# nextpyp/spr_pick

Hardware: AMD Instinct MI355X
Metric: train_patches_per_sec (higher is better)
Workload: dtype f32; 1 GPU; BASELINE configs[1]: ssdn --noise_style gaussian --noise_value var, joint mode, 64x64 patches from 4 synthetic 1024x1024 micrographs, batch 32 per GPU, alpha 0.75, tau 0.01, Adam; fp32 MFMA convolutions (Winograd F(2x2,3x3) for the wide 3x3 layers); per_gpu_batch=32, global_batch=32, patch=64, parallelism=single GPU

## Files before the change

### spr_pick_amd/csrc/gemm1x1.hip

```cpp
#include "gemm1x1.h"

#include <type_traits>

#include "conv_dev.h"

namespace {

constexpr int kTP = 256;
constexpr int kXS = kTP + 16;
constexpr int kKC = 32;
constexpr int kLdw = sprk::kGemm1x1Ldw;
constexpr int kWInstr = kKC * kLdw / 256;
static_assert(kKC * kLdw % 256 == 0 && kXS % 32 == 16 && kLdw % 32 == 16, "LDS layout");

struct G1Args {
    const float *x, *wT, *scp, *shp;
    float *y;
    int N, K, Cn, HW;
    int rows, nblkN;
    int act, hasSc, hasSh;
    int steps, nch, c0last;
    int tilesPerImg, nTiles, nh, xcd;
};

template <int NB>
__global__ __launch_bounds__(256) void gemm1x1_kernel(const G1Args a) {
    extern __shared__ __attribute__((aligned(16))) float smem[];
    constexpr int NTT = NB * 6;
    constexpr int stageFloats = kKC * kXS + NB * kKC * kLdw;
    const int tid = threadIdx.x, lane = tid & 63;
    const int wave = __builtin_amdgcn_readfirstlane(tid >> 6);
    const int l15 = lane & 15, lq = lane >> 4;
    const int G = gridDim.x;

    auto decode = [&](int r, int &t, int &h) {
        const int b = blockIdx.x;
        if (a.xcd) {
            const int j = b >> 3;
            h = j % a.nh;
            t = r * (G / a.nh) + (j / a.nh) * 8 + (b & 7);
        } else {
            const int it = r * G + b;
            t = it / a.nh;
            h = it - t * a.nh;
        }
        t = __builtin_amdgcn_readfirstlane(t);
        h = __builtin_amdgcn_readfirstlane(h);
        return t < a.nTiles;
    };
    const rsrc_t wr = make_rsrc(a.wT);
    auto issue = [&](int t, int h, int ci, int b) {
        const int n = __builtin_amdgcn_readfirstlane(t / a.tilesPerImg), p0 = (t - n * a.tilesPerImg) * kTP;
        float *xs = smem + b * stageFloats;
        float *ws = xs + kKC * kXS;
        const rsrc_t xr = make_rsrc(a.x + (long)n * a.K * a.HW);
        const int xv = min(p0 + lane * 4, a.HW - 4) * 4;
        const int r0 = ci * kKC;
#pragma unroll
        for (int i = 0; i < kKC / 4; ++i) {
            const int r = r0 + wave + 4 * i;
            const int ch = r < a.K ? r : a.c0last;
            bdma16(xr, xv, ch * a.HW * 4, xs + (wave + 4 * i) * kXS);
        }
        const int valid = min(kKC, a.rows - r0) * kLdw * 4 - 16;
#pragma unroll
        for (int i0 = 0; i0 < NB * kWInstr; i0 += 4) {
            const int i = min(i0 + wave, NB * kWInstr - 1);
            const int nbi = i / kWInstr, ii = i - nbi * kWInstr;
            const int nb = min(h * NB + nbi, a.nblkN - 1);
            bdma16(wr, min(ii * 1024 + lane * 16, valid), (nb * a.rows + r0) * (kLdw * 4), ws + nbi * (kKC * kLdw) + ii * 256);
        }
    };
    constexpr int kDmaPerWave = kKC / 4 + (NB * kWInstr + 3) / 4;

    int t, h;
    bool ok = decode(0, t, h);
    if (!ok) return;
    issue(t, h, 0, 0);
    const int abase = lds_addr(smem) + (lq * kXS + wave * 64 + l15) * 4;
    const int bbase = lds_addr(smem + kKC * kXS) + (lq * kLdw + l15) * 4;
    int g = 0;
    for (int r = 0; ok; ++r) {
        int tn, hn;
        const bool okn = decode(r + 1, tn, hn);
        const int n = __builtin_amdgcn_readfirstlane(t / a.tilesPerImg), p0 = (t - n * a.tilesPerImg) * kTP;
        const int pix = p0 + wave * 64 + lq * 4;
        float vsc[NTT], vsh[NTT];
#pragma unroll
        for (int j = 0; j < NTT; ++j) {
            const int idx = min(h * (NB * 96) + j * 16 + l15, a.Cn - 1);
            vsc[j] = a.scp[a.hasSc ? idx : 0];
            vsh[j] = a.shp[a.hasSh ? idx : 0];
        }
        f32x4 acc[4][NTT];
#pragma unroll
        for (int mt = 0; mt < 4; ++mt)
#pragma unroll
            for (int j = 0; j < NTT; ++j) acc[mt][j] = f32x4{0.f, 0.f, 0.f, 0.f};

        for (int ci = 0; ci < a.nch; ++ci, ++g) {
            if (ci > 0 || r == 0) asm volatile("s_waitcnt vmcnt(0)" ::: "memory");
            lds_only_barrier();
            const bool lastc = ci + 1 == a.nch;
            const int nq = min(kKC / 4, a.steps - ci * (kKC / 4));
            const int sa = abase + (g & 1) * (stageFloats * 4), sb = bbase + (g & 1) * (stageFloats * 4);
            float a0[4], b0[NTT], a1[4], b1[NTT];
            auto ld = [&](float (&av)[4], float (&bv)[NTT], int q) {
                lds_cfp ap = lds_f(sa + q * (4 * kXS * 4));
#pragma unroll
                for (int mt = 0; mt < 4; ++mt) av[mt] = ap[16 * mt];
                lds_cfp bp = lds_f(sb + q * (4 * kLdw * 4));
#pragma unroll
                for (int j = 0; j < NTT; ++j) bv[j] = bp[(j / 6) * (kKC * kLdw) + 16 * (j % 6)];
            };
            auto mm = [&](const float (&av)[4], const float (&bv)[NTT]) {
#pragma unroll
                for (int mt = 0; mt < 4; ++mt)
#pragma unroll
                    for (int j = 0; j < NTT; ++j)
                        acc[mt][j] = __builtin_amdgcn_mfma_f32_16x16x4f32(av[mt], bv[j], acc[mt][j], 0, 0, 0);
            };
            const int last = nq - 1;
            ld(a0, b0, 0);
            ld(a1, b1, min(1, last));
            {
                const bool own = !lastc || !okn;
                issue(own ? t : tn, own ? h : hn, lastc ? 0 : ci + 1, (g + 1) & 1);
            }
            mm(a0, b0);
#pragma unroll
            for (int i = 0; i < kDmaPerWave; ++i) {
                __builtin_amdgcn_sched_group_barrier(0x008, 4 * NTT / kDmaPerWave, 0);
                __builtin_amdgcn_sched_group_barrier(0x020, 1, 0);
            }
            for (int q = 1; q + 1 < nq; q += 2) {
                ld(a0, b0, q + 1);
                mm(a1, b1);
                ld(a1, b1, min(q + 2, last));
                mm(a0, b0);
            }
            if (!(nq & 1)) mm(a1, b1);
        }
        asm volatile("s_waitcnt vmcnt(0)" ::: "memory");
#pragma unroll
        for (int j = 0; j < NTT; ++j) asm volatile("" : "+v"(vsc[j]), "+v"(vsh[j]));
        auto stores = [&](auto actc) {
            constexpr int ACT = decltype(actc)::value;
#pragma unroll
            for (int j = 0; j < NTT; ++j) {
                const int co = h * (NB * 96) + j * 16 + l15;
                if (co >= a.Cn) continue;
                const float sc = a.hasSc ? vsc[j] : 1.f, sh = vsh[j];
                float *yc = a.y + ((long)n * a.Cn + co) * a.HW + pix;
#pragma unroll
                for (int mt = 0; mt < 4; ++mt) {
                    if (pix + 16 * mt >= a.HW) continue;
                    const f32x4 c = acc[mt][j];
                    float v[4];
#pragma unroll
                    for (int e = 0; e < 4; ++e) v[e] = apply_act(c[e] * sc + sh, ACT);
                    *reinterpret_cast<float4 *>(yc + 16 * mt) = make_float4(v[0], v[1], v[2], v[3]);
                }
            }
        };
        if (a.act == SPRK_ACT_LEAKY)
            stores(std::integral_constant<int, SPRK_ACT_LEAKY>{});
        else if (a.act == SPRK_ACT_RELU)
            stores(std::integral_constant<int, SPRK_ACT_RELU>{});
        else
            stores(std::integral_constant<int, SPRK_ACT_NONE>{});
        t = tn;
        h = hn;
        ok = okn;
    }
}

inline int slabs_per_item(int nblkN) { return nblkN >= 2 ? 2 : 1; }

template <int NB>
int launch(const G1Args &a, int grid, hipStream_t s) {
    const size_t lds = 2 * (size_t)(kKC * kXS + NB * kKC * kLdw) * sizeof(float);
    if (int rc = sprk::lds_optin(gemm1x1_kernel<NB>, lds, "gemm1x1")) return rc;
    hipLaunchKernelGGL(gemm1x1_kernel<NB>, dim3(grid), dim3(256), lds, s, a);
    return SPRK_OK;
}

}

namespace sprk {

std::atomic<long> g_gemm1x1_launches{0};
std::atomic<int> g_gemm1x1_on{1};

bool gemm1x1_fits(int N, int K, int HW) {
    return K >= kGemm1x1MinK && HW >= 4 && HW % 4 == 0 && (long)K * HW * 4 < (1L << 31) &&
           (long)N * cdiv(HW, kTP) < (1L << 28);
}

int gemm1x1_grid(int N, int HW, int nblkN) {
    const int nh = cdiv(nblkN, slabs_per_item(nblkN));
    const long items = (long)N * cdiv(HW, kTP) * nh;
    int G = (int)std::min<long>(items, num_cus());
    if (G >= 8 * nh) G -= G % (8 * nh);
    return std::max(G, 1);
}

int gemm1x1_run(const Gemm1x1Call &c, hipStream_t s) {
    SPRK_REQUIRE(gemm1x1_fits(c.N, c.K, c.HW) && c.ldw == kLdw && c.rows == cdiv(c.K, 16) * 16 && c.nblkN >= 1 &&
                     c.nblkN == cdiv(c.Cn, 96) && (long)c.nblkN * c.rows * kLdw * 4 < (1L << 31),
                 "gemm1x1: call outside the kernel's limits");
    const int NB = slabs_per_item(c.nblkN);
    G1Args a{};
    a.x = c.x; a.wT = c.wT; a.y = c.y;
    a.scp = c.scale ? c.scale : c.zeros;
    a.shp = c.scale ? c.shift : (c.bias ? c.bias : c.zeros);
    a.hasSc = c.scale != nullptr;
    a.hasSh = (c.scale || c.bias) ? 1 : 0;
    a.N = c.N; a.K = c.K; a.Cn = c.Cn; a.HW = c.HW;
    a.rows = c.rows; a.nblkN = c.nblkN;
    a.act = c.act;
    a.steps = cdiv(c.K, 4);
    a.nch = cdiv(a.steps, kKC / 4);
    a.c0last = (c.K - 1) / 16 * 16;
    a.tilesPerImg = cdiv(c.HW, kTP);
    a.nTiles = c.N * a.tilesPerImg;
    a.nh = cdiv(c.nblkN, NB);
    const int grid = gemm1x1_grid(c.N, c.HW, c.nblkN);
    a.xcd = (grid % (8 * a.nh) == 0) ? 1 : 0;
    if (int rc = NB == 2 ? launch<2>(a, grid, s) : launch<1>(a, grid, s)) return rc;
    g_gemm1x1_launches.fetch_add(1, std::memory_order_relaxed);
    return SPRK_OK;
}

}
```

### spr_pick_amd/csrc/mask1x1.hip

```cpp
#include "mask1x1.h"

#include "conv_dev.h"

namespace {

constexpr int kTP = 128;
constexpr int kMaxSteps = 30;
constexpr int kTabEntries = kMaxSteps + 2;

struct M1Args {
    const float *gy, *wT, *mask;
    float *gin;
    int N, K, Cn, HW;
    int CK, R4, rows, ldw;
    int act, steps, tilesPerImg, nTiles;
};

using i32x2 = __attribute__((ext_vector_type(2))) int;
typedef const __attribute__((address_space(3))) i32x2 *lds_ci2p;

template <int NT>
__global__ __launch_bounds__(256) void mask1x1_kernel(const M1Args a) {
    extern __shared__ __attribute__((aligned(16))) float smem[];
    i32x2 *tab = reinterpret_cast<i32x2 *>(smem);
    float *w_lds = smem + kTabEntries * 4 * 2;
    const int wFloats = a.rows * a.ldw;
    float *stage = w_lds + wFloats;
    const int stageFloats = a.K * kTP;

    const int tid = threadIdx.x, lane = tid & 63;
    const int wave = __builtin_amdgcn_readfirstlane(tid >> 6);
    const int l15 = lane & 15, lq = lane >> 4;
    const int nb = blockIdx.y;
    const long HW = a.HW;

    {
        const float *wsrc = a.wT + (long)nb * wFloats;
        const int total4 = wFloats >> 2;
        for (int gi = wave; gi * 64 < total4; gi += 4) {
            const int idx = gi * 64 + lane;
            if (idx < total4) dma16(wsrc + idx * 4, w_lds + gi * 256);
        }
    }
    auto issue = [&](int t, int b) {
        const int n = t / a.tilesPerImg, p0 = (t - n * a.tilesPerImg) * kTP;
        const int chl = lane >> 5;
        const int px = min(p0 + (lane & 31) * 4, a.HW - 4);
        const float *src = a.gy + (long)n * a.K * HW + px;
        float *dst = stage + b * stageFloats;
        for (int c = wave * 2; c < a.K; c += 8) {
            const int ch = c + chl;
            if (ch < a.K) dma16(src + (long)ch * HW, dst + c * kTP);
        }
    };
    int t = blockIdx.x;
    issue(t, 0);
    if (tid < kTabEntries * 4) {
        const int s = min(tid >> 2, a.steps - 1), l = tid & 3;
        int c0 = 0, ci = 0, q = s;
        for (;;) {
            const int nkq = (min(a.CK, a.K - c0) + 3) >> 2;
            if (q < nkq) break;
            q -= nkq;
            c0 += a.CK;
            ++ci;
        }
        const int cke = min(a.CK, a.K - c0), kk = 4 * q + l;
        tab[tid] = i32x2{(c0 + (kk < cke ? kk : 0)) * (kTP * 4), (ci * a.R4 + kk) * (a.ldw * 4)};
    }
    const int abase = lds_addr(stage) + (wave * 32 + l15) * 4;
    const int bbase = lds_addr(w_lds) + l15 * 4;
    lds_ci2p tp = (lds_ci2p)(__SIZE_TYPE__)(unsigned)lds_addr(tab + lq);
    const bool leaky = a.act == SPRK_ACT_LEAKY;

    asm volatile("s_waitcnt vmcnt(0)" ::: "memory");
    for (int i = 0; t < a.nTiles; t += gridDim.x, ++i) {
        lds_only_barrier();
        if (t + (int)gridDim.x < a.nTiles) issue(t + gridDim.x, (i + 1) & 1);
        const int n = t / a.tilesPerImg, p0 = (t - n * a.tilesPerImg) * kTP;
        const int pix = p0 + wave * 32 + lq * 4;
        float4 mk[2][NT];
#pragma unroll
        for (int nt = 0; nt < NT; ++nt) {
            const int co = min(nb * (NT * 16) + nt * 16 + l15, a.Cn - 1);
            const float *mp = a.mask + ((long)n * a.Cn + co) * HW;
#pragma unroll
            for (int mt = 0; mt < 2; ++mt) mk[mt][nt] = *reinterpret_cast<const float4 *>(mp + min(pix + 16 * mt, a.HW - 4));
        }
        f32x4 acc[2][NT];
#pragma unroll
        for (int mt = 0; mt < 2; ++mt)
#pragma unroll
            for (int nt = 0; nt < NT; ++nt) acc[mt][nt] = f32x4{0.f, 0.f, 0.f, 0.f};
        const int sa = abase + (i & 1) * stageFloats * 4;
        float av[2], bv[NT];
        i32x2 e1 = tp[4];
        {
            const i32x2 e0 = tp[0];
            lds_cfp ap = lds_f(sa + e0.x);
            av[0] = ap[0];
            av[1] = ap[16];
            lds_cfp bp = lds_f(bbase + e0.y);
#pragma unroll
            for (int nt = 0; nt < NT; ++nt) bv[nt] = bp[16 * nt];
        }
        for (int s = 0; s < a.steps; ++s) {
            const i32x2 e2 = tp[(s + 2) * 4];
            float an[2], bn[NT];
            lds_cfp ap = lds_f(sa + e1.x);
            an[0] = ap[0];
            an[1] = ap[16];
            lds_cfp bp = lds_f(bbase + e1.y);
#pragma unroll
            for (int nt = 0; nt < NT; ++nt) bn[nt] = bp[16 * nt];
#pragma unroll
            for (int mt = 0; mt < 2; ++mt)
#pragma unroll
                for (int nt = 0; nt < NT; ++nt)
                    acc[mt][nt] = __builtin_amdgcn_mfma_f32_16x16x4f32(av[mt], bv[nt], acc[mt][nt], 0, 0, 0);
            av[0] = an[0];
            av[1] = an[1];
#pragma unroll
            for (int nt = 0; nt < NT; ++nt) bv[nt] = bn[nt];
            e1 = e2;
        }
        asm volatile("s_waitcnt vmcnt(0)" ::: "memory");
#pragma unroll
        for (int nt = 0; nt < NT; ++nt)
#pragma unroll
            for (int mt = 0; mt < 2; ++mt)
                asm volatile("" : "+v"(mk[mt][nt].x), "+v"(mk[mt][nt].y), "+v"(mk[mt][nt].z), "+v"(mk[mt][nt].w));
#pragma unroll
        for (int nt = 0; nt < NT; ++nt) {
            const int co = nb * (NT * 16) + nt * 16 + l15;
            if (co >= a.Cn) continue;
#pragma unroll
            for (int mt = 0; mt < 2; ++mt) {
                if (pix + 16 * mt >= a.HW) continue;
                const f32x4 c = acc[mt][nt];
                const float4 m = mk[mt][nt];
                float4 v = make_float4(c[0] + 0.f, c[1] + 0.f, c[2] + 0.f, c[3] + 0.f);
                v.x = m.x > 0.f ? v.x : (leaky ? v.x * kLeak : 0.f);
                v.y = m.y > 0.f ? v.y : (leaky ? v.y * kLeak : 0.f);
                v.z = m.z > 0.f ? v.z : (leaky ? v.z * kLeak : 0.f);
                v.w = m.w > 0.f ? v.w : (leaky ? v.w * kLeak : 0.f);
                *reinterpret_cast<float4 *>(a.gin + ((long)n * a.Cn + co) * HW + pix + 16 * mt) = v;
            }
        }
    }
}

template <int NT>
int launch(const M1Args &a, dim3 grid, size_t lds, hipStream_t s) {
    if (int rc = sprk::lds_optin(mask1x1_kernel<NT>, lds, "mask1x1")) return rc;
    hipLaunchKernelGGL(mask1x1_kernel<NT>, grid, dim3(256), lds, s, a);
    return SPRK_OK;
}

}

namespace sprk {

int mask1x1_steps(int K, int CK) {
    if (K < 1 || K > kMask1x1MaxK || CK < 1) return 0;
    int steps = 0;
    for (int c0 = 0; c0 < K; c0 += CK) steps += (std::min(CK, K - c0) + 3) >> 2;
    return steps <= kMaxSteps ? steps : 0;
}

int mask1x1_run(const Mask1x1Call &c, hipStream_t s) {
    M1Args a{};
    a.gy = c.gy; a.wT = c.wT; a.mask = c.mask; a.gin = c.gin;
    a.N = c.N; a.K = c.K; a.Cn = c.Cn; a.HW = c.HW;
    a.CK = c.CK; a.R4 = c.R4; a.rows = c.rows; a.ldw = c.ldw;
    a.act = c.act;
    a.steps = mask1x1_steps(c.K, c.CK);
    a.tilesPerImg = cdiv(c.HW, kTP);
    a.nTiles = c.N * a.tilesPerImg;
    SPRK_REQUIRE(a.steps > 0 && c.HW >= 4 && c.HW % 4 == 0 && (long)c.N * a.tilesPerImg < (1L << 30) &&
                     (c.rows * c.ldw) % 4 == 0 && (c.act == SPRK_ACT_LEAKY || c.act == SPRK_ACT_RELU),
                 "mask1x1: call outside the kernel's limits");
    const size_t lds = ((size_t)kTabEntries * 8 + (size_t)c.rows * c.ldw + 2 * (size_t)c.K * kTP) * sizeof(float);
    SPRK_REQUIRE(lds <= 160 * 1024, "mask1x1: %zu bytes of LDS", lds);
    int wgs = std::max(1, num_cus() / c.nblkN);
    if (wgs >= 8) wgs &= ~7;
    const dim3 grid(std::min(a.nTiles, wgs), c.nblkN);
    int rc;
    switch (c.NT) {
        case 1: rc = launch<1>(a, grid, lds, s); break;
        case 2: rc = launch<2>(a, grid, lds, s); break;
        case 3: rc = launch<3>(a, grid, lds, s); break;
        case 4: rc = launch<4>(a, grid, lds, s); break;
        case 6: rc = launch<6>(a, grid, lds, s); break;
        default: set_error("mask1x1: no kernel for %d channel tiles per slab", c.NT); return SPRK_EINVAL;
    }
    if (rc) return rc;
    g_mask1x1_launches.fetch_add(1, std::memory_order_relaxed);
    return SPRK_OK;
}

}
```

Baseline: 2084 patches/s.

## Split 1x1 GEMM and mask kernels across eight waves per workgroup

The gemm1x1 kernel now launches eight waves, with the two halves splitting the output channel tiles, which halves the per-wave accumulator count, and it also seeds the first MFMA with zero instead of clearing accumulators. The mask1x1 kernel halves its pixel tile and runs two independent four-wave groups per workgroup, each with its own double-buffered stage, interleaving tiles and using staggered barriers. The aim is more waves in flight and less register pressure to hide LDS and MFMA latency. The costs are more LDS per block, extra barriers, and B-operand LDS reads repeated across the wave halves. A scratch benchmark script is added.

```diff
diff --git a/scratch/head_waves_bench.py b/scratch/head_waves_bench.py
--- /dev/null
+++ b/scratch/head_waves_bench.py
@@ -0,0 +1,52 @@
+import statistics
+import sys
+
+import torch
+
+from spr_pick_amd import _lib, ops
+
+reps = int(sys.argv[1]) if len(sys.argv) > 1 else 10
+L = _lib.lib()
+S = torch.ops.sprk
+dev = torch.device("cuda:0")
+g = torch.Generator().manual_seed(1)
+N, HW = 64, 64
+
+
+def timed(fn):
+    ts = []
+    for _ in range(reps):
+        a, b = torch.cuda.Event(enable_timing=True), torch.cuda.Event(enable_timing=True)
+        a.record()
+        fn()
+        b.record()
+        torch.cuda.synchronize()
+        ts.append(a.elapsed_time(b) * 1e3)
+    return ts
+
+
+def rnd(*shape, scale=1.0):
+    return (torch.randn(*shape, generator=g) * scale).to(dev)
+
+
+for name, K, Cout, kind in (("gemm1x1 fwd 384->384", 384, 384, "fwd"), ("gemm1x1 fwd 384->96", 384, 96, "fwd"),
+                            ("gemm1x1 bwd 384->384", 384, 384, "bwd"), ("mask1x1 bwd 96->384", 96, 384, "mask")):
+    x = rnd(N, K, HW, HW)
+    if kind == "fwd":
+        w, b = rnd(Cout, K, 1, 1, scale=K ** -0.5), rnd(Cout)
+        geom = ops.make_geom(x, None, w, False, 1, 1, (0, 0, 0, 0))
+        fn = lambda: ops.conv2d_forward(x, None, w, geom, bias=b, act=ops.ACT_LEAKY)
+    else:
+        w = rnd(K, Cout, 1, 1, scale=K ** -0.5)
+        mask = rnd(N, Cout, HW, HW) if kind == "mask" else None
+        geom = ops.make_geom(torch.empty(N, Cout, HW, HW, device=dev), None, w, False, 1, 1, (0, 0, 0, 0))
+        fn = lambda: S.conv2d_bwd_data(x, w, ops.geom_list(geom), mask, ops.ACT_LEAKY if kind == "mask" else ops.ACT_NONE, None)
+    n0 = L.sprk_gemm1x1_launch_count(), L.sprk_mask1x1_launch_count()
+    fn()
+    torch.cuda.synchronize()
+    took = L.sprk_gemm1x1_launch_count() - n0[0], L.sprk_mask1x1_launch_count() - n0[1]
+    ts = timed(fn)
+    print("%-22s launches (gemm1x1, mask1x1) %s  median %.1f us  min %.1f  max %.1f  (%.1f TF at the minimum)" % (
+        name, took, statistics.median(ts), min(ts), max(ts), 2.0 * N * HW * HW * K * Cout / min(ts) * 1e-6), flush=True)
+    del x, w, fn
+    torch.cuda.empty_cache()
diff --git a/spr_pick_amd/csrc/gemm1x1.hip b/spr_pick_amd/csrc/gemm1x1.hip
--- a/spr_pick_amd/csrc/gemm1x1.hip
+++ b/spr_pick_amd/csrc/gemm1x1.hip
@@ -9,9 +9,10 @@
 constexpr int kTP = 256;
 constexpr int kXS = kTP + 16;
 constexpr int kKC = 32;
+constexpr int kNW = 8;
 constexpr int kLdw = sprk::kGemm1x1Ldw;
 constexpr int kWInstr = kKC * kLdw / 256;
-static_assert(kKC * kLdw % 256 == 0 && kXS % 32 == 16 && kLdw % 32 == 16, "LDS layout");
+static_assert(kKC % kNW == 0 && kKC * kLdw % 256 == 0 && kXS % 32 == 16 && kLdw % 32 == 16, "LDS layout");
 
 struct G1Args {
     const float *x, *wT, *scp, *shp;
@@ -24,12 +25,13 @@
 };
 
 template <int NB>
-__global__ __launch_bounds__(256) void gemm1x1_kernel(const G1Args a) {
+__global__ __launch_bounds__(kNW * 64) void gemm1x1_kernel(const G1Args a) {
     extern __shared__ __attribute__((aligned(16))) float smem[];
-    constexpr int NTT = NB * 6;
+    constexpr int NTT = NB * 3;
     constexpr int stageFloats = kKC * kXS + NB * kKC * kLdw;
     const int tid = threadIdx.x, lane = tid & 63;
     const int wave = __builtin_amdgcn_readfirstlane(tid >> 6);
+    const int wq = wave & 3, wh = wave >> 2;
     const int l15 = lane & 15, lq = lane >> 4;
     const int G = gridDim.x;
 
@@ -57,46 +59,42 @@
         const int xv = min(p0 + lane * 4, a.HW - 4) * 4;
         const int r0 = ci * kKC;
 #pragma unroll
-        for (int i = 0; i < kKC / 4; ++i) {
-            const int r = r0 + wave + 4 * i;
+        for (int i = 0; i < kKC / kNW; ++i) {
+            const int r = r0 + wave + kNW * i;
             const int ch = r < a.K ? r : a.c0last;
-            bdma16(xr, xv, ch * a.HW * 4, xs + (wave + 4 * i) * kXS);
+            bdma16(xr, xv, ch * a.HW * 4, xs + (wave + kNW * i) * kXS);
         }
         const int valid = min(kKC, a.rows - r0) * kLdw * 4 - 16;
 #pragma unroll
-        for (int i0 = 0; i0 < NB * kWInstr; i0 += 4) {
+        for (int i0 = 0; i0 < NB * kWInstr; i0 += kNW) {
             const int i = min(i0 + wave, NB * kWInstr - 1);
             const int nbi = i / kWInstr, ii = i - nbi * kWInstr;
             const int nb = min(h * NB + nbi, a.nblkN - 1);
             bdma16(wr, min(ii * 1024 + lane * 16, valid), (nb * a.rows + r0) * (kLdw * 4), ws + nbi * (kKC * kLdw) + ii * 256);
         }
     };
-    constexpr int kDmaPerWave = kKC / 4 + (NB * kWInstr + 3) / 4;
+    constexpr int kDmaPerWave = kKC / kNW + (NB * kWInstr + kNW - 1) / kNW;
 
     int t, h;
     bool ok = decode(0, t, h);
     if (!ok) return;
     issue(t, h, 0, 0);
-    const int abase = lds_addr(smem) + (lq * kXS + wave * 64 + l15) * 4;
-    const int bbase = lds_addr(smem + kKC * kXS) + (lq * kLdw + l15) * 4;
+    const int abase = lds_addr(smem) + (lq * kXS + wq * 64 + l15) * 4;
+    const int bbase = lds_addr(smem + kKC * kXS) + (wh * NTT / 6 * (kKC * kLdw) + lq * kLdw + wh * NTT % 6 * 16 + l15) * 4;
     int g = 0;
     for (int r = 0; ok; ++r) {
         int tn, hn;
         const bool okn = decode(r + 1, tn, hn);
         const int n = __builtin_amdgcn_readfirstlane(t / a.tilesPerImg), p0 = (t - n * a.tilesPerImg) * kTP;
-        const int pix = p0 + wave * 64 + lq * 4;
+        const int pix = p0 + wq * 64 + lq * 4;
         float vsc[NTT], vsh[NTT];
 #pragma unroll
         for (int j = 0; j < NTT; ++j) {
-            const int idx = min(h * (NB * 96) + j * 16 + l15, a.Cn - 1);
+            const int idx = min(h * (NB * 96) + (wh * NTT + j) * 16 + l15, a.Cn - 1);
             vsc[j] = a.scp[a.hasSc ? idx : 0];
             vsh[j] = a.shp[a.hasSh ? idx : 0];
         }
         f32x4 acc[4][NTT];
-#pragma unroll
-        for (int mt = 0; mt < 4; ++mt)
-#pragma unroll
-            for (int j = 0; j < NTT; ++j) acc[mt][j] = f32x4{0.f, 0.f, 0.f, 0.f};
 
         for (int ci = 0; ci < a.nch; ++ci, ++g) {
             if (ci > 0 || r == 0) asm volatile("s_waitcnt vmcnt(0)" ::: "memory");
@@ -111,35 +109,40 @@
                 for (int mt = 0; mt < 4; ++mt) av[mt] = ap[16 * mt];
                 lds_cfp bp = lds_f(sb + q * (4 * kLdw * 4));
 #pragma unroll
-                for (int j = 0; j < NTT; ++j) bv[j] = bp[(j / 6) * (kKC * kLdw) + 16 * (j % 6)];
+                for (int j = 0; j < NTT; ++j) bv[j] = bp[16 * j];
             };
-            auto mm = [&](const float (&av)[4], const float (&bv)[NTT]) {
+            auto mm = [&](const float (&av)[4], const float (&bv)[NTT], auto first) {
 #pragma unroll
                 for (int mt = 0; mt < 4; ++mt)
 #pragma unroll
                     for (int j = 0; j < NTT; ++j)
-                        acc[mt][j] = __builtin_amdgcn_mfma_f32_16x16x4f32(av[mt], bv[j], acc[mt][j], 0, 0, 0);
+                        acc[mt][j] = __builtin_amdgcn_mfma_f32_16x16x4f32(
+                            av[mt], bv[j], decltype(first)::value ? f32x4{0.f, 0.f, 0.f, 0.f} : acc[mt][j], 0, 0, 0);
             };
             const int last = nq - 1;
             ld(a0, b0, 0);
             ld(a1, b1, min(1, last));
-            {
+            auto step0 = [&](auto first) {
                 const bool own = !lastc || !okn;
                 issue(own ? t : tn, own ? h : hn, lastc ? 0 : ci + 1, (g + 1) & 1);
-            }
-            mm(a0, b0);
-#pragma unroll
-            for (int i = 0; i < kDmaPerWave; ++i) {
-                __builtin_amdgcn_sched_group_barrier(0x008, 4 * NTT / kDmaPerWave, 0);
-                __builtin_amdgcn_sched_group_barrier(0x020, 1, 0);
-            }
+                mm(a0, b0, first);
+#pragma unroll
+                for (int i = 0; i < kDmaPerWave; ++i) {
+                    __builtin_amdgcn_sched_group_barrier(0x008, 4 * NTT / kDmaPerWave, 0);
+                    __builtin_amdgcn_sched_group_barrier(0x020, 1, 0);
+                }
+            };
+            if (ci == 0)
+                step0(std::true_type{});
+            else
+                step0(std::false_type{});
             for (int q = 1; q + 1 < nq; q += 2) {
                 ld(a0, b0, q + 1);
-                mm(a1, b1);
+                mm(a1, b1, std::false_type{});
                 ld(a1, b1, min(q + 2, last));
-                mm(a0, b0);
+                mm(a0, b0, std::false_type{});
             }
-            if (!(nq & 1)) mm(a1, b1);
+            if (!(nq & 1)) mm(a1, b1, std::false_type{});
         }
         asm volatile("s_waitcnt vmcnt(0)" ::: "memory");
 #pragma unroll
@@ -148,7 +151,7 @@
             constexpr int ACT = decltype(actc)::value;
 #pragma unroll
             for (int j = 0; j < NTT; ++j) {
-                const int co = h * (NB * 96) + j * 16 + l15;
+                const int co = h * (NB * 96) + (wh * NTT + j) * 16 + l15;
                 if (co >= a.Cn) continue;
                 const float sc = a.hasSc ? vsc[j] : 1.f, sh = vsh[j];
                 float *yc = a.y + ((long)n * a.Cn + co) * a.HW + pix;
@@ -181,7 +184,7 @@
 int launch(const G1Args &a, int grid, hipStream_t s) {
     const size_t lds = 2 * (size_t)(kKC * kXS + NB * kKC * kLdw) * sizeof(float);
     if (int rc = sprk::lds_optin(gemm1x1_kernel<NB>, lds, "gemm1x1")) return rc;
-    hipLaunchKernelGGL(gemm1x1_kernel<NB>, dim3(grid), dim3(256), lds, s, a);
+    hipLaunchKernelGGL(gemm1x1_kernel<NB>, dim3(grid), dim3(kNW * 64), lds, s, a);
     return SPRK_OK;
 }
 
diff --git a/spr_pick_amd/csrc/mask1x1.hip b/spr_pick_amd/csrc/mask1x1.hip
--- a/spr_pick_amd/csrc/mask1x1.hip
+++ b/spr_pick_amd/csrc/mask1x1.hip
@@ -4,7 +4,7 @@
 
 namespace {
 
-constexpr int kTP = 128;
+constexpr int kTP = 64;
 constexpr int kMaxSteps = 30;
 constexpr int kTabEntries = kMaxSteps + 2;
 
@@ -20,41 +20,43 @@
 typedef const __attribute__((address_space(3))) i32x2 *lds_ci2p;
 
 template <int NT>
-__global__ __launch_bounds__(256) void mask1x1_kernel(const M1Args a) {
+__global__ __launch_bounds__(512) void mask1x1_kernel(const M1Args a) {
     extern __shared__ __attribute__((aligned(16))) float smem[];
     i32x2 *tab = reinterpret_cast<i32x2 *>(smem);
     float *w_lds = smem + kTabEntries * 4 * 2;
     const int wFloats = a.rows * a.ldw;
-    float *stage = w_lds + wFloats;
     const int stageFloats = a.K * kTP;
 
     const int tid = threadIdx.x, lane = tid & 63;
-    const int wave = __builtin_amdgcn_readfirstlane(tid >> 6);
+    const int wave8 = __builtin_amdgcn_readfirstlane(tid >> 6);
+    const int grp = wave8 >> 2, wave = wave8 & 3;
     const int l15 = lane & 15, lq = lane >> 4;
-    const int nb = blockIdx.y;
+    const int nb = blockIdx.y, G = gridDim.x;
     const long HW = a.HW;
+    float *stage = w_lds + wFloats + grp * 2 * stageFloats;
 
     {
         const float *wsrc = a.wT + (long)nb * wFloats;
         const int total4 = wFloats >> 2;
-        for (int gi = wave; gi * 64 < total4; gi += 4) {
+        for (int gi = wave8; gi * 64 < total4; gi += 8) {
             const int idx = gi * 64 + lane;
             if (idx < total4) dma16(wsrc + idx * 4, w_lds + gi * 256);
         }
     }
     auto issue = [&](int t, int b) {
         const int n = t / a.tilesPerImg, p0 = (t - n * a.tilesPerImg) * kTP;
-        const int chl = lane >> 5;
-        const int px = min(p0 + (lane & 31) * 4, a.HW - 4);
+        const int chl = lane >> 4;
+        const int px = min(p0 + (lane & 15) * 4, a.HW - 4);
         const float *src = a.gy + (long)n * a.K * HW + px;
         float *dst = stage + b * stageFloats;
-        for (int c = wave * 2; c < a.K; c += 8) {
+        for (int c = wave * 4; c < a.K; c += 16) {
             const int ch = c + chl;
             if (ch < a.K) dma16(src + (long)ch * HW, dst + c * kTP);
         }
     };
-    int t = blockIdx.x;
-    issue(t, 0);
+    int t = blockIdx.x + grp * G;
+    const int rounds = ((a.nTiles - (int)blockIdx.x + G - 1) / G + 1) >> 1;
+    if (t < a.nTiles) issue(t, 0);
     if (tid < kTabEntries * 4) {
         const int s = min(tid >> 2, a.steps - 1), l = tid & 3;
         int c0 = 0, ci = 0, q = s;
@@ -68,92 +70,83 @@
         const int cke = min(a.CK, a.K - c0), kk = 4 * q + l;
         tab[tid] = i32x2{(c0 + (kk < cke ? kk : 0)) * (kTP * 4), (ci * a.R4 + kk) * (a.ldw * 4)};
     }
-    const int abase = lds_addr(stage) + (wave * 32 + l15) * 4;
+    const int abase = lds_addr(stage) + (wave * 16 + l15) * 4;
     const int bbase = lds_addr(w_lds) + l15 * 4;
     lds_ci2p tp = (lds_ci2p)(__SIZE_TYPE__)(unsigned)lds_addr(tab + lq);
     const bool leaky = a.act == SPRK_ACT_LEAKY;
+    const int half = a.steps >> 1;
 
     asm volatile("s_waitcnt vmcnt(0)" ::: "memory");
-    for (int i = 0; t < a.nTiles; t += gridDim.x, ++i) {
+    if (grp) lds_only_barrier();
+    for (int i = 0; i < rounds; ++i, t += 2 * G) {
         lds_only_barrier();
-        if (t + (int)gridDim.x < a.nTiles) issue(t + gridDim.x, (i + 1) & 1);
+        if (t >= a.nTiles) {
+            lds_only_barrier();
+            continue;
+        }
+        if (t + 2 * G < a.nTiles) issue(t + 2 * G, (i + 1) & 1);
         const int n = t / a.tilesPerImg, p0 = (t - n * a.tilesPerImg) * kTP;
-        const int pix = p0 + wave * 32 + lq * 4;
-        float4 mk[2][NT];
+        const int pix = p0 + wave * 16 + lq * 4;
+        float4 mk[NT];
 #pragma unroll
         for (int nt = 0; nt < NT; ++nt) {
             const int co = min(nb * (NT * 16) + nt * 16 + l15, a.Cn - 1);
-            const float *mp = a.mask + ((long)n * a.Cn + co) * HW;
+            mk[nt] = *reinterpret_cast<const float4 *>(a.mask + ((long)n * a.Cn + co) * HW + min(pix, a.HW - 4));
+        }
+        f32x4 acc[NT];
 #pragma unroll
-            for (int mt = 0; mt < 2; ++mt) mk[mt][nt] = *reinterpret_cast<const float4 *>(mp + min(pix + 16 * mt, a.HW - 4));
-        }
-        f32x4 acc[2][NT];
-#pragma unroll
-        for (int mt = 0; mt < 2; ++mt)
-#pragma unroll
-            for (int nt = 0; nt < NT; ++nt) acc[mt][nt] = f32x4{0.f, 0.f, 0.f, 0.f};
+        for (int nt = 0; nt < NT; ++nt) acc[nt] = f32x4{0.f, 0.f, 0.f, 0.f};
         const int sa = abase + (i & 1) * stageFloats * 4;
-        float av[2], bv[NT];
+        float av, bv[NT];
         i32x2 e1 = tp[4];
         {
             const i32x2 e0 = tp[0];
-            lds_cfp ap = lds_f(sa + e0.x);
-            av[0] = ap[0];
-            av[1] = ap[16];
+            av = lds_f(sa + e0.x)[0];
             lds_cfp bp = lds_f(bbase + e0.y);
 #pragma unroll
             for (int nt = 0; nt < NT; ++nt) bv[nt] = bp[16 * nt];
         }
         for (int s = 0; s < a.steps; ++s) {
+            if (s == half) lds_only_barrier();
             const i32x2 e2 = tp[(s + 2) * 4];
-            float an[2], bn[NT];
-            lds_cfp ap = lds_f(sa + e1.x);
-            an[0] = ap[0];
-            an[1] = ap[16];
+            float an, bn[NT];
+            an = lds_f(sa + e1.x)[0];
             lds_cfp bp = lds_f(bbase + e1.y);
 #pragma unroll
             for (int nt = 0; nt < NT; ++nt) bn[nt] = bp[16 * nt];
 #pragma unroll
-            for (int mt = 0; mt < 2; ++mt)
-#pragma unroll
-                for (int nt = 0; nt < NT; ++nt)
-                    acc[mt][nt] = __builtin_amdgcn_mfma_f32_16x16x4f32(av[mt], bv[nt], acc[mt][nt], 0, 0, 0);
-            av[0] = an[0];
-            av[1] = an[1];
+            for (int nt = 0; nt < NT; ++nt) acc[nt] = __builtin_amdgcn_mfma_f32_16x16x4f32(av, bv[nt], acc[nt], 0, 0, 0);
+            av = an;
 #pragma unroll
             for (int nt = 0; nt < NT; ++nt) bv[nt] = bn[nt];
             e1 = e2;
         }
         asm volatile("s_waitcnt vmcnt(0)" ::: "memory");
 #pragma unroll
-        for (int nt = 0; nt < NT; ++nt)
+        for (int nt = 0; nt < NT; ++nt) asm volatile("" : "+v"(mk[nt].x), "+v"(mk[nt].y), "+v"(mk[nt].z), "+v"(mk[nt].w));
+        if (pix < a.HW) {
 #pragma unroll
-            for (int mt = 0; mt < 2; ++mt)
-                asm volatile("" : "+v"(mk[mt][nt].x), "+v"(mk[mt][nt].y), "+v"(mk[mt][nt].z), "+v"(mk[mt][nt].w));
-#pragma unroll
-        for (int nt = 0; nt < NT; ++nt) {
-            const int co = nb * (NT * 16) + nt * 16 + l15;
-            if (co >= a.Cn) continue;
-#pragma unroll
-            for (int mt = 0; mt < 2; ++mt) {
-                if (pix + 16 * mt >= a.HW) continue;
-                const f32x4 c = acc[mt][nt];
-                const float4 m = mk[mt][nt];
+            for (int nt = 0; nt < NT; ++nt) {
+                const int co = nb * (NT * 16) + nt * 16 + l15;
+                if (co >= a.Cn) continue;
+                const f32x4 c = acc[nt];
+                const float4 m = mk[nt];
                 float4 v = make_float4(c[0] + 0.f, c[1] + 0.f, c[2] + 0.f, c[3] + 0.f);
                 v.x = m.x > 0.f ? v.x : (leaky ? v.x * kLeak : 0.f);
                 v.y = m.y > 0.f ? v.y : (leaky ? v.y * kLeak : 0.f);
                 v.z = m.z > 0.f ? v.z : (leaky ? v.z * kLeak : 0.f);
                 v.w = m.w > 0.f ? v.w : (leaky ? v.w * kLeak : 0.f);
-                *reinterpret_cast<float4 *>(a.gin + ((long)n * a.Cn + co) * HW + pix + 16 * mt) = v;
+                *reinterpret_cast<float4 *>(a.gin + ((long)n * a.Cn + co) * HW + pix) = v;
             }
         }
     }
+    if (!grp) lds_only_barrier();
 }
 
 template <int NT>
 int launch(const M1Args &a, dim3 grid, size_t lds, hipStream_t s) {
     if (int rc = sprk::lds_optin(mask1x1_kernel<NT>, lds, "mask1x1")) return rc;
-    hipLaunchKernelGGL(mask1x1_kernel<NT>, grid, dim3(256), lds, s, a);
+    hipLaunchKernelGGL(mask1x1_kernel<NT>, grid, dim3(512), lds, s, a);
     return SPRK_OK;
 }
 
@@ -180,7 +173,7 @@
     SPRK_REQUIRE(a.steps > 0 && c.HW >= 4 && c.HW % 4 == 0 && (long)c.N * a.tilesPerImg < (1L << 30) &&
                      (c.rows * c.ldw) % 4 == 0 && (c.act == SPRK_ACT_LEAKY || c.act == SPRK_ACT_RELU),
                  "mask1x1: call outside the kernel's limits");
-    const size_t lds = ((size_t)kTabEntries * 8 + (size_t)c.rows * c.ldw + 2 * (size_t)c.K * kTP) * sizeof(float);
+    const size_t lds = ((size_t)kTabEntries * 8 + (size_t)c.rows * c.ldw + 4 * (size_t)c.K * kTP) * sizeof(float);
     SPRK_REQUIRE(lds <= 160 * 1024, "mask1x1: %zu bytes of LDS", lds);
     int wgs = std::max(1, num_cus() / c.nblkN);
     if (wgs >= 8) wgs &= ~7;
```

Result: no change. 2097 patches/s (median of 6 runs) (+0.6%).
